# Apokleos/kata-xpu-device-plugin

Measured on NVIDIA H100. Metric: pci.ids parse GB/s (x1000 text + 2^20-key join); device lookups/s reported beside it, higher is better.
Workload: dtype u8

## Files before the change

kata-xpu-device-plugin_b200/csrc/pciids5.cu:

```cuda
#pragma once
#include "exchange.cuh"
#include "parse_common.cuh"

namespace kxparse5 {

using namespace kxparse;

constexpr int STAGES5 = 3;
constexpr int RCH5_MAX = 8;
constexpr int RES_WARPS = 8;

struct WarpSmem5 {
    alignas(16) uint8_t stage[STAGES5][STG_BYTES];
    alignas(8) unsigned long long bar[STAGES5];
};

struct Params5 {
    const uint8_t *text;
    unsigned long long n, base;
    uint32_t num_chunks;
    uint32_t tma_limit;
    uint32_t rch;
    uint32_t num_ranges;
    unsigned long long *range_state;
    uint32_t *lead;
    unsigned long long *range_carry;
    uint32_t *tasks;
    KxTableDev tab;
    unsigned long long carry_in;
    uint32_t task_ctas;
    int xa_on;
    uint32_t *xa_done;
    kxx::XaParams xa;
};


__device__ __forceinline__ void nl_masks(uint32_t st, uint32_t lane, uint32_t n_rel, uint32_t k7f, uint32_t k0a, uint32_t k80,
                                         uint32_t (&nl)[2], uint32_t &rawnl) {
    const uint32_t swz = (lane >> 2) & 1u;
    rawnl = 0;
#pragma unroll
    for (int h = 0; h < 2; h++) {
        const uint32_t o = (uint32_t)h * HALF + lane * 32u;
        const uint4 va = lds128(st + o + 16u * swz);
        const uint4 vb = lds128(st + o + 16u * (swz ^ 1u));
        const uint32_t ma = nl_mask16(va, k7f, k0a, k80), mb = nl_mask16(vb, k7f, k0a, k80);
        const uint32_t m2 = ma | (mb << 16);
        uint32_t mm = __funnelshift_l(m2, m2, swz << 4);
        rawnl |= mm;
        if (n_rel <= (uint32_t)CW) mm &= n_rel > o + 1u ? (n_rel - o - 1u >= 32u ? 0xffffffffu : ((1u << (n_rel - o - 1u)) - 1u)) : 0u;
        nl[h] = mm;
    }
}

__device__ __forceinline__ uint32_t tops_of(uint32_t lp, uint32_t mm) {
    uint32_t tm = 0;
    while (mm) {
        const uint32_t bit = mm & (0u - mm);
        mm ^= bit;
        const uint32_t c0 = lds8(lp + (31u - (uint32_t)__clz((int)bit)));
        if (c0 != 9u && c0 != 35u) tm |= bit;
    }
    return tm;
}

__device__ __forceinline__ void tops_of2(uint32_t lp0, uint32_t m0, uint32_t m1, uint32_t &t0, uint32_t &t1) {
    t0 = t1 = 0;
    while (m0 | m1) {
        const uint32_t b0 = m0 & (0u - m0), b1 = m1 & (0u - m1);
        m0 ^= b0;
        m1 ^= b1;
        const uint32_t c0 = lds8(lp0 + (31u - (uint32_t)__clz((int)b0)));
        const uint32_t c1 = lds8(lp0 + (uint32_t)HALF + (31u - (uint32_t)__clz((int)b1)));
        if (c0 != 9u && c0 != 35u) t0 |= b0;
        if (c1 != 9u && c1 != 35u) t1 |= b1;
    }
}

__device__ __forceinline__ uint32_t devs_of(uint32_t lp, uint32_t mm) {
    uint32_t km = 0;
    while (mm) {
        const uint32_t bit = mm & (0u - mm);
        mm ^= bit;
        const uint32_t a = lp + (31u - (uint32_t)__clz((int)bit));
        if (lds8(a) == 9u && lds8(a + 1u) != 9u) km |= bit;
    }
    return km;
}

__global__ void __launch_bounds__(NT, 4) parse_kernel_v5(const Params5 P) {
    extern __shared__ __align__(128) uint8_t smem_raw[];
    WarpSmem5 *W = reinterpret_cast<WarpSmem5 *>(smem_raw);
    uint32_t lane = threadIdx.x & 31u;
    const uint32_t w = threadIdx.x >> 5;
    asm volatile("" : "+r"(lane));
    const uint32_t lt_mask = (1u << lane) - 1u;

    if (lane == 0) {
        for (int s = 0; s < STAGES5; s++) mbar_init(&W[w].bar[s], 1);
        asm volatile("fence.mbarrier_init.release.cluster;" ::: "memory");
    }
    uint32_t tk = 0;
    if (lane == 0) tk = atomicAdd(&P.tab.counters[KX_C_TICKET], 1u);
    uint32_t r = __shfl_sync(0xffffffffu, tk, 0);
    if (r >= P.num_ranges) return;

    uint32_t a_stage0 = smem_u32(smem_raw) + w * (uint32_t)sizeof(WarpSmem5);
    asm volatile("" : "+r"(a_stage0));
    const uint32_t a_bar0 = a_stage0 + (uint32_t)offsetof(WarpSmem5, bar);

    uint32_t k7f = 0x7f7f7f7fu, k0a = 0x0a0a0a0au, k80 = 0x80808080u;
    asm volatile("" : "+r"(k7f), "+r"(k0a), "+r"(k80));

    const unsigned long long pol = l2_evict_first_policy();
    auto issue = [&](uint32_t g, uint32_t s) {
        if (g < P.tma_limit) {
            mbar_expect_tx_a(a_bar0 + 8u * s, STG_BYTES);
            tma_load_a(a_stage0 + s * (uint32_t)STG_BYTES, P.text + (unsigned long long)g * CW, STG_BYTES, a_bar0 + 8u * s, pol);
        }
    };
    const uint32_t rch = P.rch;
    bool staged = false;

    uint32_t phase_bits = 0, s = 0;
    uint32_t nfresh = 0;
    for (;;) {
        uint32_t tk2 = 0, r_next = 0xffffffffu;
        bool have_next = false;
        if (lane == 0) tk2 = atomicAdd(&P.tab.counters[KX_C_TICKET], 1u);
        uint32_t rc_x = 0, rc_g = 0;
        if (r == 0u) {
            rc_x = LS_PUB | (((P.carry_in & CV_HAS_TOP) && (P.carry_in & CV_VOK)) ? (LS_TOP | LS_VOK) : 0u);
            rc_g = 0xffffffffu;
        }
        uint32_t lead = r == 0u ? 0u : rch;
        const bool table_dead = *reinterpret_cast<volatile uint32_t *>(&P.tab.counters[KX_C_OVERFLOW]) != 0u;
        const uint32_t gb = r * rch;
        const uint32_t cnt = P.num_chunks - gb < rch ? P.num_chunks - gb : rch;
        if (!staged && lane == 0) {
            for (uint32_t j = 0; j < (uint32_t)STAGES5 && j < cnt; j++) issue(gb + j, (s + j) % (uint32_t)STAGES5);
        }
        staged = false;
        for (uint32_t i = 0; i < cnt; i++) {
            if (!have_next && rch > (uint32_t)STAGES5 && i + (uint32_t)STAGES5 >= rch) {
                r_next = __shfl_sync(0xffffffffu, tk2, 0);
                have_next = true;
            }
            const uint32_t g = gb + i;
            const uint32_t st = a_stage0 + s * (uint32_t)STG_BYTES;
            const unsigned long long cbase = P.base + (unsigned long long)g * CW;
            uint32_t n_rel = CW + 1;
            if (g < P.tma_limit) {
                const uint32_t bar = a_bar0 + 8u * s, par = (phase_bits >> s) & 1u;
                while (!mbar_try_a(bar, par)) {
                }
                phase_bits ^= 1u << s;
            } else {
                n_rel = stage_chunk_manual(P.text, P.n, g, lane, W[w].stage[s]);
            }

            uint32_t nl[2], th[2], rawnl;
            nl_masks(st, lane, n_rel, k7f, k0a, k80, nl, rawnl);
            tops_of2(st + lane * 32u + 1u, nl[0], nl[1], th[0], th[1]);

            uint32_t linfo0 = P_NONE, linfo1 = P_NONE;
            bool any_alive = (g == 0u) || (rc_x & LS_VOK) != 0u;
            {
                uint32_t t0 = th[0], t1 = th[1];
                while (t0 | t1) {
                    const bool second = t0 == 0u;
                    const uint32_t tmv = second ? t1 : t0;
                    const uint32_t bit = tmv & (0u - tmv);
                    if (second) t1 = tmv ^ bit; else t0 = tmv ^ bit;
                    const uint32_t p = (second ? (uint32_t)HALF : 0u) + lane * 32u + 1u + (31u - (uint32_t)__clz((int)bit));
                    uint32_t val;
                    const bool ok = hex4_swar(lds32_unaligned(st + p), val);
                    const unsigned long long line_g = cbase + p;
                    bool alive = ok;
                    if (ok) {
                        const unsigned long long vf = P.tab.vendor_first[val];
                        if (line_g < vf) atomicMin(&P.tab.vendor_first[val], line_g);
                        alive = line_g <= vf;
                    }
                    any_alive |= alive;
                    const uint32_t info = (alive ? 0x80000000u : 0u) | ((ok ? val : 0u) << 15) | p;
                    if (second) linfo1 = info; else linfo0 = info;
                }
            }
            const uint32_t bal0 = __ballot_sync(0xffffffffu, th[0] != 0u);
            const uint32_t bal1 = __ballot_sync(0xffffffffu, th[1] != 0u);
            uint32_t last1;
            if (!__any_sync(0xffffffffu, any_alive)) {
                const uint32_t bl = bal1 ? bal1 : bal0;
                last1 = __shfl_sync(0xffffffffu, bal1 ? linfo1 : linfo0, bl ? 31 - __clz((int)bl) : 0);
                if (bl == 0u) last1 = P_NONE;
            } else {
                uint32_t kh[2];
                kh[0] = th[0] | devs_of(st + lane * 32u + 1u, nl[0] & ~th[0]);
                kh[1] = th[1] | devs_of(st + (uint32_t)HALF + lane * 32u + 1u, nl[1] & ~th[1]);
                if (table_dead) { kh[0] = th[0]; kh[1] = th[1]; }

                uint32_t base_info = P_NONE;
                if (g == 0u && n_rel > 0u) {
                    const uint32_t c0 = lds8(st), c1 = lds8(st + 1u);
                    if (c0 != (uint32_t)'#' && c0 != (uint32_t)'\t') {
                        uint32_t val;
                        const bool ok = hex4_swar(lds32_unaligned(st), val);
                        bool alive = ok;
                        if (ok) {
                            const unsigned long long vf = P.tab.vendor_first[val];
                            if (lane == 0 && cbase < vf) atomicMin(&P.tab.vendor_first[val], cbase);
                            alive = cbase <= vf;
                        }
                        base_info = (alive ? 0x80000000u : 0u) | ((ok ? val : 0u) << 15);
                    } else if (c0 == (uint32_t)'\t' && c1 != (uint32_t)'\t') {
                        uint32_t dv;
                        if (lane == 0 && !table_dead && (P.carry_in & CV_HAS_TOP) && (P.carry_in & CV_VOK) && hex4_swar(lds32_unaligned(st + 1u), dv))
                            table_fold(P.tab, (((uint32_t)(P.carry_in >> 44) & 0xffffu) << 16) | dv, cbase, P.carry_in & CV_ANCHOR_MASK, nfresh);
                    }
                }
                linfo0 = linfo1 = P_NONE;
                {
                    uint32_t t0 = th[0], t1 = th[1];
                    while (t0 | t1) {
                        const bool second = t0 == 0u;
                        const uint32_t tmv = second ? t1 : t0;
                        const uint32_t bit = tmv & (0u - tmv);
                        const uint32_t rest = tmv ^ bit;
                        if (second) t1 = rest; else t0 = rest;
                        const uint32_t pbase = (second ? (uint32_t)HALF : 0u) + lane * 32u + 1u;
                        const uint32_t p = pbase + (31u - (uint32_t)__clz((int)bit));
                        uint32_t val;
                        const bool ok = hex4_swar(lds32_unaligned(st + p), val);
                        const unsigned long long line_g = cbase + p;
                        const bool alive = ok && line_g <= P.tab.vendor_first[val];
                        if (alive) {
                            const uint32_t nxt = rest & (0u - rest);
                            const uint32_t seg = (second ? kh[1] & ~th[1] : kh[0] & ~th[0]) & ~(bit | (bit - 1u)) & (nxt ? nxt - 1u : 0xffffffffu);
                            fold_lines(P.tab, st, cbase, seg, pbase, val << 16, line_g, nfresh);
                        }
                        const uint32_t info = (alive ? 0x80000000u : 0u) | ((ok ? val : 0u) << 15) | p;
                        if (second) linfo1 = info; else linfo0 = info;
                    }
                }
                const uint32_t pre0 = kh[0] & ~th[0] & (th[0] ? (th[0] & (0u - th[0])) - 1u : 0xffffffffu);
                const uint32_t pre1 = kh[1] & ~th[1] & (th[1] ? (th[1] & (0u - th[1])) - 1u : 0xffffffffu);
                const uint32_t s0 = bal0 & lt_mask, s1 = bal1 & lt_mask;
                const uint32_t x0 = __shfl_sync(0xffffffffu, linfo0, s0 ? 31 - __clz((int)s0) : 0);
                const uint32_t l0 = __shfl_sync(0xffffffffu, linfo0, bal0 ? 31 - __clz((int)bal0) : 0);
                const uint32_t x1 = __shfl_sync(0xffffffffu, linfo1, s1 ? 31 - __clz((int)s1) : 0);
                const uint32_t l1 = __shfl_sync(0xffffffffu, linfo1, bal1 ? 31 - __clz((int)bal1) : 0);
                const uint32_t last0 = bal0 ? l0 : base_info;
                const uint32_t cin0 = s0 ? x0 : base_info;
                const uint32_t cin1 = s1 ? x1 : last0;
                last1 = bal1 ? l1 : last0;
                if (cin0 != P_NONE && (cin0 >> 31))
                    fold_lines(P.tab, st, cbase, pre0, lane * 32u + 1u, ((cin0 >> 15) & 0xffffu) << 16, cbase + (cin0 & 0x7fffu), nfresh);
                if (cin1 != P_NONE && (cin1 >> 31))
                    fold_lines(P.tab, st, cbase, pre1, (uint32_t)HALF + lane * 32u + 1u, ((cin1 >> 15) & 0xffffu) << 16, cbase + (cin1 & 0x7fffu), nfresh);
                const uint32_t hw0 = cin0 == P_NONE ? pre0 : 0u;
                const uint32_t hw1 = cin1 == P_NONE ? pre1 : 0u;
                if (rc_x & LS_VOK) {
                    uint32_t key_hi = ((rc_x >> 12) & 0xffffu) << 16;
                    unsigned long long anchor = P.base + (unsigned long long)rc_g * CW + (rc_x & 0xfffu);
                    if (rc_g == 0xffffffffu) {
                        key_hi = ((uint32_t)(P.carry_in >> 44) & 0xffffu) << 16;
                        anchor = P.carry_in & CV_ANCHOR_MASK;
                    }
                    if ((hw0 | hw1) != 0u && P.tab.vendor_first[key_hi >> 16] >= anchor) {
                        fold_lines(P.tab, st, cbase, hw0, lane * 32u + 1u, key_hi, anchor, nfresh);
                        fold_lines(P.tab, st, cbase, hw1, (uint32_t)HALF + lane * 32u + 1u, key_hi, anchor, nfresh);
                    }
                }
                flush_fresh(P.tab, nfresh);
            }
            if (last1 != P_NONE) {
                if (rc_x == 0u) lead = i + 1u;
                rc_x = LS_PUB | LS_TOP | ((last1 >> 31) ? LS_VOK : 0u) | (((last1 >> 15) & 0xffffu) << 12) | (last1 & 0xfffu);
                rc_g = g;
            }
            if ((bal0 | bal1) == 0u && n_rel > (uint32_t)CW && __reduce_or_sync(0xffffffffu, rawnl) == 0u && lane == 0)
                atomicOr(&P.tab.counters[KX_C_LONGLINE_HINT], 1u);

            __syncwarp();
            {
                const uint32_t fi = i + (uint32_t)STAGES5;
                uint32_t fg = 0xffffffffu;
                if (fi < rch) {
                    fg = g + (uint32_t)STAGES5;
                } else if (rch > (uint32_t)STAGES5 && cnt == rch && r_next < P.num_ranges) {
                    fg = r_next * rch + (fi - rch);
                    staged = true;
                }
                if (lane == 0) issue(fg, s);
            }
            s = s == (uint32_t)STAGES5 - 1u ? 0u : s + 1u;
        }
        if (lane == 0) {
            unsigned long long v = ST_NONE;
            if (rc_x != 0u) {
                if (rc_g == 0xffffffffu)
                    v = ST_PREFIX | P.carry_in;
                else
                    v = ST_PREFIX | CV_HAS_TOP | ((rc_x & LS_VOK) ? CV_VOK : 0ull) | ((unsigned long long)((rc_x >> 12) & 0xffffu) << 44) |
                        ((P.base + (unsigned long long)rc_g * CW + (rc_x & 0xfffu)) & CV_ANCHOR_MASK);
            }
            P.range_state[r] = v;
            P.lead[r] = lead < cnt ? lead : cnt;
        }
        if (!have_next) r_next = __shfl_sync(0xffffffffu, tk2, 0);
        r = r_next;
        if (r >= P.num_ranges) break;
    }
}

constexpr uint32_t XA_CTAS = 64;

__global__ void __launch_bounds__(256) resolve_ranges_kernel(const Params5 P) {
    const uint32_t rr = blockIdx.x * blockDim.x + threadIdx.x;
    const uint32_t lane = threadIdx.x & 31u;
    const uint32_t rr0 = rr - lane;
    if (rr0 >= P.num_ranges) return;
    const bool live = rr < P.num_ranges;
    const uint32_t nlead = live ? P.lead[rr] : 0u;
    const unsigned long long own = live ? P.range_state[rr] : ST_NONE;
    const uint32_t pm = __ballot_sync(0xffffffffu, (own & ST_MASK) == ST_PREFIX);
    const uint32_t below = pm & ((1u << lane) - 1u);
    const unsigned long long from_warp = __shfl_sync(0xffffffffu, own, below ? 31 - __clz((int)below) : 0);
    unsigned long long warp_in = 0;
    const uint32_t first_p = pm ? (uint32_t)__ffs((int)pm) - 1u : 32u;
    const bool want = __any_sync(0xffffffffu, nlead != 0u && lane <= first_p);
    if (want) {
        long long q0 = (long long)rr0 - 32;
        for (;;) {
            const long long q = q0 + lane;
            const unsigned long long sv = q >= 0 ? P.range_state[q] : (q == -1 ? (ST_PREFIX | P.carry_in) : ST_NONE);
            const uint32_t m = __ballot_sync(0xffffffffu, (sv & ST_MASK) == ST_PREFIX);
            if (m) {
                warp_in = __shfl_sync(0xffffffffu, sv, 31 - __clz((int)m));
                break;
            }
            q0 -= 32;
        }
    }
    const unsigned long long carry = (below ? from_warp : warp_in) & ~ST_MASK;
    const bool alive = nlead != 0u && (carry & CV_HAS_TOP) && (carry & CV_VOK) &&
                       P.tab.vendor_first[(uint32_t)(carry >> 44) & 0xffffu] >= (carry & CV_ANCHOR_MASK);
    const uint32_t mine = alive ? nlead : 0u;
    uint32_t incl = mine;
#pragma unroll
    for (int d = 1; d < 32; d <<= 1) {
        const uint32_t y = __shfl_up_sync(0xffffffffu, incl, d);
        if (lane >= (uint32_t)d) incl += y;
    }
    const uint32_t tot = __shfl_sync(0xffffffffu, incl, 31);
    uint32_t at0 = 0;
    if (lane == 0 && tot) at0 = atomicAdd(&P.tab.counters[KX_C_DEFER], tot);
    at0 = __shfl_sync(0xffffffffu, at0, 0);
    if (!alive) return;
    P.range_carry[rr] = carry;
    const uint32_t at = at0 + incl - mine;
    for (uint32_t j = 0; j < nlead; j++) P.tasks[at + j] = rr * P.rch + j;
}

__global__ void __launch_bounds__(RES_WARPS * 32) resolve_chunks_kernel(const Params5 P) {
    __shared__ __align__(16) uint8_t stg[RES_WARPS][STG_BYTES];
    __shared__ __align__(8) unsigned long long bars[RES_WARPS];
    __shared__ uint16_t plist[RES_WARPS][704];
    if (blockIdx.x >= P.task_ctas) {
        kxx::xa_push_slice(P.xa, (blockIdx.x - P.task_ctas) * blockDim.x + threadIdx.x, XA_CTAS * blockDim.x);
        __syncthreads();
        if (threadIdx.x == 0) {
            kx_fence_sys();
            const uint32_t prev = atomicAdd(P.xa_done, 1u);
            if (prev == XA_CTAS - 1u) {
                *P.xa_done = 0u;
                kx_fence_sys();
                kxx::xa_finish(P.xa);
            }
        }
        return;
    }
    const uint32_t lane = threadIdx.x & 31u, w = threadIdx.x >> 5;
    const uint32_t lt_mask = (1u << lane) - 1u;
    uint32_t k7f = 0x7f7f7f7fu, k0a = 0x0a0a0a0au, k80 = 0x80808080u;
    asm volatile("" : "+r"(k7f), "+r"(k0a), "+r"(k80));
    const uint32_t st = smem_u32(stg[w]), bar = smem_u32(&bars[w]);
    if (lane == 0) {
        mbar_init(&bars[w], 1);
        asm volatile("fence.mbarrier_init.release.cluster;" ::: "memory");
    }
    __syncwarp();
    const unsigned long long pol = l2_evict_first_policy();
    const uint32_t n_tasks = P.tab.counters[KX_C_DEFER];
    uint32_t par = 0, nfresh = 0;
    const bool small_tab = P.tab.cap <= (1u << 20);
    uint32_t it = 0;
    for (uint32_t t = blockIdx.x * RES_WARPS + w; t < n_tasks; t += P.task_ctas * RES_WARPS, it++) {
        if ((it & 3u) == 0u && *reinterpret_cast<volatile uint32_t *>(&P.tab.counters[KX_C_OVERFLOW]) != 0u) break;
        const uint32_t gg = P.tasks[t];
        uint32_t n_rel = CW + 1;
        if (gg < P.tma_limit) {
            if (lane == 0) {
                mbar_expect_tx_a(bar, STG_BYTES);
                tma_load_a(st, P.text + (unsigned long long)gg * CW, STG_BYTES, bar, pol);
            }
            while (!mbar_try_a(bar, par)) {
            }
            par ^= 1u;
        } else {
            n_rel = stage_chunk_manual(P.text, P.n, gg, lane, stg[w]);
        }
        const unsigned long long cc = P.range_carry[gg / P.rch];
        const uint32_t key_hi = ((uint32_t)(cc >> 44) & 0xffffu) << 16;
        const unsigned long long anchor = cc & CV_ANCHOR_MASK;
        uint32_t kh[2], th[2], rawnl;
        chunk_masks(st, lane, n_rel, k7f, k0a, k80, kh, th, rawnl);
        const uint32_t bal0 = __ballot_sync(0xffffffffu, th[0] != 0u);
        const uint32_t bal1 = __ballot_sync(0xffffffffu, th[1] != 0u);
        const uint32_t pre0 = kh[0] & ~th[0] & (th[0] ? (th[0] & (0u - th[0])) - 1u : 0xffffffffu);
        const uint32_t pre1 = kh[1] & ~th[1] & (th[1] ? (th[1] & (0u - th[1])) - 1u : 0xffffffffu);
        const unsigned long long cbase = P.base + (unsigned long long)gg * CW;
        const uint32_t m0 = (bal0 & lt_mask) == 0u ? pre0 : 0u;
        const uint32_t m1 = (bal0 == 0u && (bal1 & lt_mask) == 0u) ? pre1 : 0u;
        const uint32_t mine = (uint32_t)__popc(m0) + (uint32_t)__popc(m1);
        uint32_t incl = mine;
#pragma unroll
        for (int d = 1; d < 32; d <<= 1) {
            const uint32_t y = __shfl_up_sync(0xffffffffu, incl, d);
            if (lane >= (uint32_t)d) incl += y;
        }
        const uint32_t total = __shfl_sync(0xffffffffu, incl, 31);
        {
            uint32_t idx = incl - mine;
            for (uint32_t m = m0; m; m &= m - 1u) plist[w][idx++] = (uint16_t)(lane * 32u + 1u + (uint32_t)__ffs((int)m) - 1u);
            for (uint32_t m = m1; m; m &= m - 1u) plist[w][idx++] = (uint16_t)((uint32_t)HALF + lane * 32u + 1u + (uint32_t)__ffs((int)m) - 1u);
        }
        __syncwarp();
        if (small_tab) {
            for (uint32_t i = lane; i < total; i += 64u) {
                uint32_t d0, d1 = 0;
                const uint32_t p0 = plist[w][i], p1 = i + 32u < total ? plist[w][i + 32u] : 0u;
                bool v0 = hex4_swar(lds32_unaligned(st + p0 + 1u), d0);
                bool v1 = i + 32u < total && hex4_swar(lds32_unaligned(st + p1 + 1u), d1);
                uint32_t q0 = p0, q1 = p1;
                if (!v0 && v1) { d0 = d1; q0 = p1; v0 = true; v1 = false; }
                if (v0) table_fold_claim2(P.tab, key_hi | d0, cbase + q0, anchor, v1, key_hi | d1, cbase + q1, anchor, nfresh);
            }
        } else {
            for (uint32_t i = lane; i < total; i += 32u) {
                const uint32_t p = plist[w][i];
                uint32_t dv;
                if (hex4_swar(lds32_unaligned(st + p + 1u), dv)) table_fold(P.tab, key_hi | dv, cbase + p, anchor, nfresh);
            }
        }
        __syncwarp();
        flush_fresh(P.tab, nfresh);
    }
}

}
```

Measured before the change: 2479.

## Batch three chunks per TMA copy with two stages, drop cross-range prefetch

Each TMA bulk copy now loads three consecutive chunks plus a trailing overlap into one stage buffer, and only two stage buffers are kept per warp. The aim is fewer, larger bulk copies and fewer mbarrier waits per chunk. The prefetch of the next range's first chunks before the current range finishes is removed, so each range starts with an exposed load. The larger shared-memory footprint lowers the launch-bounds occupancy hint from 4 CTAs to 2, and a whole copy group falls back to manual staging if any of its chunks lies past the TMA limit.

After: 2565 (median of 6 runs). +3.5%, better.

```diff
diff --git a/kata-xpu-device-plugin_b200/csrc/pciids5.cu b/kata-xpu-device-plugin_b200/csrc/pciids5.cu
--- a/kata-xpu-device-plugin_b200/csrc/pciids5.cu
+++ b/kata-xpu-device-plugin_b200/csrc/pciids5.cu
@@ -6,12 +6,15 @@
 
 using namespace kxparse;
 
-constexpr int STAGES5 = 3;
-constexpr int RCH5_MAX = 8;
+constexpr int CPC5 = 3;
+constexpr int STAGES5 = 2;
+constexpr int CTAS5 = 2;
+constexpr int COPY5 = CPC5 * CW + TRAIL;
+constexpr int RCH5_MAX = CPC5 * STAGES5;
 constexpr int RES_WARPS = 8;
 
 struct WarpSmem5 {
-    alignas(16) uint8_t stage[STAGES5][STG_BYTES];
+    alignas(16) uint8_t stage[STAGES5][COPY5];
     alignas(8) unsigned long long bar[STAGES5];
 };
 
@@ -88,7 +91,7 @@
     return km;
 }
 
-__global__ void __launch_bounds__(NT, 4) parse_kernel_v5(const Params5 P) {
+__global__ void __launch_bounds__(NT, CTAS5) parse_kernel_v5(const Params5 P) {
     extern __shared__ __align__(128) uint8_t smem_raw[];
     WarpSmem5 *W = reinterpret_cast<WarpSmem5 *>(smem_raw);
     uint32_t lane = threadIdx.x & 31u;
@@ -113,20 +116,21 @@
     asm volatile("" : "+r"(k7f), "+r"(k0a), "+r"(k80));
 
     const unsigned long long pol = l2_evict_first_policy();
-    auto issue = [&](uint32_t g, uint32_t s) {
-        if (g < P.tma_limit) {
-            mbar_expect_tx_a(a_bar0 + 8u * s, STG_BYTES);
-            tma_load_a(a_stage0 + s * (uint32_t)STG_BYTES, P.text + (unsigned long long)g * CW, STG_BYTES, a_bar0 + 8u * s, pol);
-        }
+    const uint32_t rch = P.rch;
+    auto copy_chunks = [](uint32_t cnt, uint32_t k) -> uint32_t {
+        return cnt - k * (uint32_t)CPC5 < (uint32_t)CPC5 ? cnt - k * (uint32_t)CPC5 : (uint32_t)CPC5;
     };
-    const uint32_t rch = P.rch;
-    bool staged = false;
+    auto issue = [&](uint32_t g0, uint32_t m, uint32_t s) {
+        if (g0 + m - 1u < P.tma_limit) {
+            mbar_expect_tx_a(a_bar0 + 8u * s, m * (uint32_t)CW + (uint32_t)TRAIL);
+            tma_load_a(a_stage0 + s * (uint32_t)COPY5, P.text + (unsigned long long)g0 * CW, m * (uint32_t)CW + (uint32_t)TRAIL, a_bar0 + 8u * s, pol);
+        }
+    };
 
     uint32_t phase_bits = 0, s = 0;
     uint32_t nfresh = 0;
     for (;;) {
-        uint32_t tk2 = 0, r_next = 0xffffffffu;
-        bool have_next = false;
+        uint32_t tk2 = 0;
         if (lane == 0) tk2 = atomicAdd(&P.tab.counters[KX_C_TICKET], 1u);
         uint32_t rc_x = 0, rc_g = 0;
         if (r == 0u) {
@@ -137,163 +141,153 @@
         const bool table_dead = *reinterpret_cast<volatile uint32_t *>(&P.tab.counters[KX_C_OVERFLOW]) != 0u;
         const uint32_t gb = r * rch;
         const uint32_t cnt = P.num_chunks - gb < rch ? P.num_chunks - gb : rch;
-        if (!staged && lane == 0) {
-            for (uint32_t j = 0; j < (uint32_t)STAGES5 && j < cnt; j++) issue(gb + j, (s + j) % (uint32_t)STAGES5);
-        }
-        staged = false;
-        for (uint32_t i = 0; i < cnt; i++) {
-            if (!have_next && rch > (uint32_t)STAGES5 && i + (uint32_t)STAGES5 >= rch) {
-                r_next = __shfl_sync(0xffffffffu, tk2, 0);
-                have_next = true;
-            }
-            const uint32_t g = gb + i;
-            const uint32_t st = a_stage0 + s * (uint32_t)STG_BYTES;
-            const unsigned long long cbase = P.base + (unsigned long long)g * CW;
-            uint32_t n_rel = CW + 1;
-            if (g < P.tma_limit) {
+        const uint32_t ncp = (cnt + (uint32_t)CPC5 - 1u) / (uint32_t)CPC5;
+        if (lane == 0) {
+            for (uint32_t j = 0; j < (uint32_t)STAGES5 && j < ncp; j++) issue(gb + j * (uint32_t)CPC5, copy_chunks(cnt, j), (s + j) % (uint32_t)STAGES5);
+        }
+        for (uint32_t k = 0; k < ncp; k++) {
+            const uint32_t g0 = gb + k * (uint32_t)CPC5, m = copy_chunks(cnt, k);
+            const bool by_tma = g0 + m - 1u < P.tma_limit;
+            if (by_tma) {
                 const uint32_t bar = a_bar0 + 8u * s, par = (phase_bits >> s) & 1u;
                 while (!mbar_try_a(bar, par)) {
                 }
                 phase_bits ^= 1u << s;
-            } else {
-                n_rel = stage_chunk_manual(P.text, P.n, g, lane, W[w].stage[s]);
-            }
-
-            uint32_t nl[2], th[2], rawnl;
-            nl_masks(st, lane, n_rel, k7f, k0a, k80, nl, rawnl);
-            tops_of2(st + lane * 32u + 1u, nl[0], nl[1], th[0], th[1]);
-
-            uint32_t linfo0 = P_NONE, linfo1 = P_NONE;
-            bool any_alive = (g == 0u) || (rc_x & LS_VOK) != 0u;
-            {
-                uint32_t t0 = th[0], t1 = th[1];
-                while (t0 | t1) {
-                    const bool second = t0 == 0u;
-                    const uint32_t tmv = second ? t1 : t0;
-                    const uint32_t bit = tmv & (0u - tmv);
-                    if (second) t1 = tmv ^ bit; else t0 = tmv ^ bit;
-                    const uint32_t p = (second ? (uint32_t)HALF : 0u) + lane * 32u + 1u + (31u - (uint32_t)__clz((int)bit));
-                    uint32_t val;
-                    const bool ok = hex4_swar(lds32_unaligned(st + p), val);
-                    const unsigned long long line_g = cbase + p;
-                    bool alive = ok;
-                    if (ok) {
-                        const unsigned long long vf = P.tab.vendor_first[val];
-                        if (line_g < vf) atomicMin(&P.tab.vendor_first[val], line_g);
-                        alive = line_g <= vf;
-                    }
-                    any_alive |= alive;
-                    const uint32_t info = (alive ? 0x80000000u : 0u) | ((ok ? val : 0u) << 15) | p;
-                    if (second) linfo1 = info; else linfo0 = info;
-                }
-            }
-            const uint32_t bal0 = __ballot_sync(0xffffffffu, th[0] != 0u);
-            const uint32_t bal1 = __ballot_sync(0xffffffffu, th[1] != 0u);
-            uint32_t last1;
-            if (!__any_sync(0xffffffffu, any_alive)) {
-                const uint32_t bl = bal1 ? bal1 : bal0;
-                last1 = __shfl_sync(0xffffffffu, bal1 ? linfo1 : linfo0, bl ? 31 - __clz((int)bl) : 0);
-                if (bl == 0u) last1 = P_NONE;
-            } else {
-                uint32_t kh[2];
-                kh[0] = th[0] | devs_of(st + lane * 32u + 1u, nl[0] & ~th[0]);
-                kh[1] = th[1] | devs_of(st + (uint32_t)HALF + lane * 32u + 1u, nl[1] & ~th[1]);
-                if (table_dead) { kh[0] = th[0]; kh[1] = th[1]; }
-
-                uint32_t base_info = P_NONE;
-                if (g == 0u && n_rel > 0u) {
-                    const uint32_t c0 = lds8(st), c1 = lds8(st + 1u);
-                    if (c0 != (uint32_t)'#' && c0 != (uint32_t)'\t') {
-                        uint32_t val;
-                        const bool ok = hex4_swar(lds32_unaligned(st), val);
-                        bool alive = ok;
-                        if (ok) {
-                            const unsigned long long vf = P.tab.vendor_first[val];
-                            if (lane == 0 && cbase < vf) atomicMin(&P.tab.vendor_first[val], cbase);
-                            alive = cbase <= vf;
-                        }
-                        base_info = (alive ? 0x80000000u : 0u) | ((ok ? val : 0u) << 15);
-                    } else if (c0 == (uint32_t)'\t' && c1 != (uint32_t)'\t') {
-                        uint32_t dv;
-                        if (lane == 0 && !table_dead && (P.carry_in & CV_HAS_TOP) && (P.carry_in & CV_VOK) && hex4_swar(lds32_unaligned(st + 1u), dv))
-                            table_fold(P.tab, (((uint32_t)(P.carry_in >> 44) & 0xffffu) << 16) | dv, cbase, P.carry_in & CV_ANCHOR_MASK, nfresh);
-                    }
-                }
-                linfo0 = linfo1 = P_NONE;
+            }
+            for (uint32_t j = 0; j < m; j++) {
+                const uint32_t i = k * (uint32_t)CPC5 + j;
+                const uint32_t g = g0 + j;
+                const uint32_t st = a_stage0 + s * (uint32_t)COPY5 + j * (uint32_t)CW;
+                const unsigned long long cbase = P.base + (unsigned long long)g * CW;
+                uint32_t n_rel = CW + 1;
+                if (!by_tma) n_rel = stage_chunk_manual(P.text, P.n, g, lane, W[w].stage[s] + j * CW);
+
+                uint32_t nl[2], th[2], rawnl;
+                nl_masks(st, lane, n_rel, k7f, k0a, k80, nl, rawnl);
+                tops_of2(st + lane * 32u + 1u, nl[0], nl[1], th[0], th[1]);
+
+                uint32_t linfo0 = P_NONE, linfo1 = P_NONE;
+                bool any_alive = (g == 0u) || (rc_x & LS_VOK) != 0u;
                 {
                     uint32_t t0 = th[0], t1 = th[1];
                     while (t0 | t1) {
                         const bool second = t0 == 0u;
                         const uint32_t tmv = second ? t1 : t0;
                         const uint32_t bit = tmv & (0u - tmv);
-                        const uint32_t rest = tmv ^ bit;
-                        if (second) t1 = rest; else t0 = rest;
-                        const uint32_t pbase = (second ? (uint32_t)HALF : 0u) + lane * 32u + 1u;
-                        const uint32_t p = pbase + (31u - (uint32_t)__clz((int)bit));
+                        if (second) t1 = tmv ^ bit; else t0 = tmv ^ bit;
+                        const uint32_t p = (second ? (uint32_t)HALF : 0u) + lane * 32u + 1u + (31u - (uint32_t)__clz((int)bit));
                         uint32_t val;
                         const bool ok = hex4_swar(lds32_unaligned(st + p), val);
                         const unsigned long long line_g = cbase + p;
-                        const bool alive = ok && line_g <= P.tab.vendor_first[val];
-                        if (alive) {
-                            const uint32_t nxt = rest & (0u - rest);
-                            const uint32_t seg = (second ? kh[1] & ~th[1] : kh[0] & ~th[0]) & ~(bit | (bit - 1u)) & (nxt ? nxt - 1u : 0xffffffffu);
-                            fold_lines(P.tab, st, cbase, seg, pbase, val << 16, line_g, nfresh);
+                        bool alive = ok;
+                        if (ok) {
+                            const unsigned long long vf = P.tab.vendor_first[val];
+                            if (line_g < vf) atomicMin(&P.tab.vendor_first[val], line_g);
+                            alive = line_g <= vf;
                         }
+                        any_alive |= alive;
                         const uint32_t info = (alive ? 0x80000000u : 0u) | ((ok ? val : 0u) << 15) | p;
                         if (second) linfo1 = info; else linfo0 = info;
                     }
                 }
-                const uint32_t pre0 = kh[0] & ~th[0] & (th[0] ? (th[0] & (0u - th[0])) - 1u : 0xffffffffu);
-                const uint32_t pre1 = kh[1] & ~th[1] & (th[1] ? (th[1] & (0u - th[1])) - 1u : 0xffffffffu);
-                const uint32_t s0 = bal0 & lt_mask, s1 = bal1 & lt_mask;
-                const uint32_t x0 = __shfl_sync(0xffffffffu, linfo0, s0 ? 31 - __clz((int)s0) : 0);
-                const uint32_t l0 = __shfl_sync(0xffffffffu, linfo0, bal0 ? 31 - __clz((int)bal0) : 0);
-                const uint32_t x1 = __shfl_sync(0xffffffffu, linfo1, s1 ? 31 - __clz((int)s1) : 0);
-                const uint32_t l1 = __shfl_sync(0xffffffffu, linfo1, bal1 ? 31 - __clz((int)bal1) : 0);
-                const uint32_t last0 = bal0 ? l0 : base_info;
-                const uint32_t cin0 = s0 ? x0 : base_info;
-                const uint32_t cin1 = s1 ? x1 : last0;
-                last1 = bal1 ? l1 : last0;
-                if (cin0 != P_NONE && (cin0 >> 31))
-                    fold_lines(P.tab, st, cbase, pre0, lane * 32u + 1u, ((cin0 >> 15) & 0xffffu) << 16, cbase + (cin0 & 0x7fffu), nfresh);
-                if (cin1 != P_NONE && (cin1 >> 31))
-                    fold_lines(P.tab, st, cbase, pre1, (uint32_t)HALF + lane * 32u + 1u, ((cin1 >> 15) & 0xffffu) << 16, cbase + (cin1 & 0x7fffu), nfresh);
-                const uint32_t hw0 = cin0 == P_NONE ? pre0 : 0u;
-                const uint32_t hw1 = cin1 == P_NONE ? pre1 : 0u;
-                if (rc_x & LS_VOK) {
-                    uint32_t key_hi = ((rc_x >> 12) & 0xffffu) << 16;
-                    unsigned long long anchor = P.base + (unsigned long long)rc_g * CW + (rc_x & 0xfffu);
-                    if (rc_g == 0xffffffffu) {
-                        key_hi = ((uint32_t)(P.carry_in >> 44) & 0xffffu) << 16;
-                        anchor = P.carry_in & CV_ANCHOR_MASK;
+                const uint32_t bal0 = __ballot_sync(0xffffffffu, th[0] != 0u);
+                const uint32_t bal1 = __ballot_sync(0xffffffffu, th[1] != 0u);
+                uint32_t last1;
+                if (!__any_sync(0xffffffffu, any_alive)) {
+                    const uint32_t bl = bal1 ? bal1 : bal0;
+                    last1 = __shfl_sync(0xffffffffu, bal1 ? linfo1 : linfo0, bl ? 31 - __clz((int)bl) : 0);
+                    if (bl == 0u) last1 = P_NONE;
+                } else {
+                    uint32_t kh[2];
+                    kh[0] = th[0] | devs_of(st + lane * 32u + 1u, nl[0] & ~th[0]);
+                    kh[1] = th[1] | devs_of(st + (uint32_t)HALF + lane * 32u + 1u, nl[1] & ~th[1]);
+                    if (table_dead) { kh[0] = th[0]; kh[1] = th[1]; }
+
+                    uint32_t base_info = P_NONE;
+                    if (g == 0u && n_rel > 0u) {
+                        const uint32_t c0 = lds8(st), c1 = lds8(st + 1u);
+                        if (c0 != (uint32_t)'#' && c0 != (uint32_t)'\t') {
+                            uint32_t val;
+                            const bool ok = hex4_swar(lds32_unaligned(st), val);
+                            bool alive = ok;
+                            if (ok) {
+                                const unsigned long long vf = P.tab.vendor_first[val];
+                                if (lane == 0 && cbase < vf) atomicMin(&P.tab.vendor_first[val], cbase);
+                                alive = cbase <= vf;
+                            }
+                            base_info = (alive ? 0x80000000u : 0u) | ((ok ? val : 0u) << 15);
+                        } else if (c0 == (uint32_t)'\t' && c1 != (uint32_t)'\t') {
+                            uint32_t dv;
+                            if (lane == 0 && !table_dead && (P.carry_in & CV_HAS_TOP) && (P.carry_in & CV_VOK) && hex4_swar(lds32_unaligned(st + 1u), dv))
+                                table_fold(P.tab, (((uint32_t)(P.carry_in >> 44) & 0xffffu) << 16) | dv, cbase, P.carry_in & CV_ANCHOR_MASK, nfresh);
+                        }
                     }
-                    if ((hw0 | hw1) != 0u && P.tab.vendor_first[key_hi >> 16] >= anchor) {
-                        fold_lines(P.tab, st, cbase, hw0, lane * 32u + 1u, key_hi, anchor, nfresh);
-                        fold_lines(P.tab, st, cbase, hw1, (uint32_t)HALF + lane * 32u + 1u, key_hi, anchor, nfresh);
+                    linfo0 = linfo1 = P_NONE;
+                    {
+                        uint32_t t0 = th[0], t1 = th[1];
+                        while (t0 | t1) {
+                            const bool second = t0 == 0u;
+                            const uint32_t tmv = second ? t1 : t0;
+                            const uint32_t bit = tmv & (0u - tmv);
+                            const uint32_t rest = tmv ^ bit;
+                            if (second) t1 = rest; else t0 = rest;
+                            const uint32_t pbase = (second ? (uint32_t)HALF : 0u) + lane * 32u + 1u;
+                            const uint32_t p = pbase + (31u - (uint32_t)__clz((int)bit));
+                            uint32_t val;
+                            const bool ok = hex4_swar(lds32_unaligned(st + p), val);
+                            const unsigned long long line_g = cbase + p;
+                            const bool alive = ok && line_g <= P.tab.vendor_first[val];
+                            if (alive) {
+                                const uint32_t nxt = rest & (0u - rest);
+                                const uint32_t seg = (second ? kh[1] & ~th[1] : kh[0] & ~th[0]) & ~(bit | (bit - 1u)) & (nxt ? nxt - 1u : 0xffffffffu);
+                                fold_lines(P.tab, st, cbase, seg, pbase, val << 16, line_g, nfresh);
+                            }
+                            const uint32_t info = (alive ? 0x80000000u : 0u) | ((ok ? val : 0u) << 15) | p;
+                            if (second) linfo1 = info; else linfo0 = info;
+                        }
                     }
+                    const uint32_t pre0 = kh[0] & ~th[0] & (th[0] ? (th[0] & (0u - th[0])) - 1u : 0xffffffffu);
+                    const uint32_t pre1 = kh[1] & ~th[1] & (th[1] ? (th[1] & (0u - th[1])) - 1u : 0xffffffffu);
+                    const uint32_t s0 = bal0 & lt_mask, s1 = bal1 & lt_mask;
+                    const uint32_t x0 = __shfl_sync(0xffffffffu, linfo0, s0 ? 31 - __clz((int)s0) : 0);
+                    const uint32_t l0 = __shfl_sync(0xffffffffu, linfo0, bal0 ? 31 - __clz((int)bal0) : 0);
+                    const uint32_t x1 = __shfl_sync(0xffffffffu, linfo1, s1 ? 31 - __clz((int)s1) : 0);
+                    const uint32_t l1 = __shfl_sync(0xffffffffu, linfo1, bal1 ? 31 - __clz((int)bal1) : 0);
+                    const uint32_t last0 = bal0 ? l0 : base_info;
+                    const uint32_t cin0 = s0 ? x0 : base_info;
+                    const uint32_t cin1 = s1 ? x1 : last0;
+                    last1 = bal1 ? l1 : last0;
+                    if (cin0 != P_NONE && (cin0 >> 31))
+                        fold_lines(P.tab, st, cbase, pre0, lane * 32u + 1u, ((cin0 >> 15) & 0xffffu) << 16, cbase + (cin0 & 0x7fffu), nfresh);
+                    if (cin1 != P_NONE && (cin1 >> 31))
+                        fold_lines(P.tab, st, cbase, pre1, (uint32_t)HALF + lane * 32u + 1u, ((cin1 >> 15) & 0xffffu) << 16, cbase + (cin1 & 0x7fffu), nfresh);
+                    const uint32_t hw0 = cin0 == P_NONE ? pre0 : 0u;
+                    const uint32_t hw1 = cin1 == P_NONE ? pre1 : 0u;
+                    if (rc_x & LS_VOK) {
+                        uint32_t key_hi = ((rc_x >> 12) & 0xffffu) << 16;
+                        unsigned long long anchor = P.base + (unsigned long long)rc_g * CW + (rc_x & 0xfffu);
+                        if (rc_g == 0xffffffffu) {
+                            key_hi = ((uint32_t)(P.carry_in >> 44) & 0xffffu) << 16;
+                            anchor = P.carry_in & CV_ANCHOR_MASK;
+                        }
+                        if ((hw0 | hw1) != 0u && P.tab.vendor_first[key_hi >> 16] >= anchor) {
+                            fold_lines(P.tab, st, cbase, hw0, lane * 32u + 1u, key_hi, anchor, nfresh);
+                            fold_lines(P.tab, st, cbase, hw1, (uint32_t)HALF + lane * 32u + 1u, key_hi, anchor, nfresh);
+                        }
+                    }
+                    flush_fresh(P.tab, nfresh);
                 }
-                flush_fresh(P.tab, nfresh);
-            }
-            if (last1 != P_NONE) {
-                if (rc_x == 0u) lead = i + 1u;
-                rc_x = LS_PUB | LS_TOP | ((last1 >> 31) ? LS_VOK : 0u) | (((last1 >> 15) & 0xffffu) << 12) | (last1 & 0xfffu);
-                rc_g = g;
-            }
-            if ((bal0 | bal1) == 0u && n_rel > (uint32_t)CW && __reduce_or_sync(0xffffffffu, rawnl) == 0u && lane == 0)
-                atomicOr(&P.tab.counters[KX_C_LONGLINE_HINT], 1u);
-
-            __syncwarp();
-            {
-                const uint32_t fi = i + (uint32_t)STAGES5;
-                uint32_t fg = 0xffffffffu;
-                if (fi < rch) {
-                    fg = g + (uint32_t)STAGES5;
-                } else if (rch > (uint32_t)STAGES5 && cnt == rch && r_next < P.num_ranges) {
-                    fg = r_next * rch + (fi - rch);
-                    staged = true;
+                if (last1 != P_NONE) {
+                    if (rc_x == 0u) lead = i + 1u;
+                    rc_x = LS_PUB | LS_TOP | ((last1 >> 31) ? LS_VOK : 0u) | (((last1 >> 15) & 0xffffu) << 12) | (last1 & 0xfffu);
+                    rc_g = g;
                 }
-                if (lane == 0) issue(fg, s);
-            }
+                if ((bal0 | bal1) == 0u && n_rel > (uint32_t)CW && __reduce_or_sync(0xffffffffu, rawnl) == 0u && lane == 0)
+                    atomicOr(&P.tab.counters[KX_C_LONGLINE_HINT], 1u);
+                __syncwarp();
+            }
+
+            if (lane == 0 && k + (uint32_t)STAGES5 < ncp) issue(gb + (k + (uint32_t)STAGES5) * (uint32_t)CPC5, copy_chunks(cnt, k + (uint32_t)STAGES5), s);
             s = s == (uint32_t)STAGES5 - 1u ? 0u : s + 1u;
         }
         if (lane == 0) {
@@ -308,8 +302,7 @@
             P.range_state[r] = v;
             P.lead[r] = lead < cnt ? lead : cnt;
         }
-        if (!have_next) r_next = __shfl_sync(0xffffffffu, tk2, 0);
-        r = r_next;
+        r = __shfl_sync(0xffffffffu, tk2, 0);
         if (r >= P.num_ranges) break;
     }
 }
```
